# RustAudio/lewton

Hardware: NVIDIA H100
Metric: Msamples/s IMDCT+window+OLA, 2048-pt long blocks (higher is better)
Workload: dtype f32

## Files before the change

lewton_b200/build.py:

```python
import os
import re
import shutil
import subprocess

HERE = os.path.dirname(os.path.abspath(__file__))
CSRC = os.path.join(HERE, "csrc")
SO = os.path.join(HERE, "liblewton_b200.so")
K_LONG_REGS = 249
SOURCES = ["lwb_api.cu", "host_objects.cuh", "path_generic.cuh", "path_long.cuh", "path_chain.cuh", "path_mixed.cuh", "path_mid.cuh",
           "tables_host.cpp", "frontend.cpp", "batcher_submit.cpp", "batcher.h", "lwb_common.h", "pcm_copy_plan.h", "kernels_generic.cuh", "kernel_long.cuh", "kernel_deal.cuh", "kernel_short.cuh", "kernel_mid.cuh", "kernel_chain.cuh", "kernel_prologue.cuh", "kernel_floor0.cuh", "floor1_eval.cuh",
           "floor1_inverse_db.inc", "Makefile"]


def _stale():
    if not os.path.exists(SO):
        return True
    t = os.path.getmtime(SO)
    deps = [os.path.join(CSRC, s) for s in SOURCES] + [os.path.join(HERE, "..", "include", h)
                                                       for h in ("lewton_b200.h", "lewton_frontend.h")]
    return any(os.path.getmtime(d) > t for d in deps)


def check_no_fma(so=SO):
    if shutil.which("cuobjdump") is None:
# ... 41 lines not shown
```

lewton_b200/csrc/host_objects.cuh:

```cuda
#pragma once

struct DevBuf {
    void *p = nullptr;
    size_t cap = 0;
};

struct Staging {
    void *h = nullptr;
    size_t cap = 0;
    cudaEvent_t ev = nullptr;
    bool pending = false;
};

struct ArenaSet {
    DevBuf coeffs, dense, pcm, kinds, ys, vqoff, vqrec;
    cudaEvent_t done = nullptr;
};
constexpr int kHostSets = 2;

struct CachedTables {
    DevTables dt;
    std::vector<float> a, b, c, w;
    std::vector<uint32_t> br;
    std::vector<void *> allocs;
// ... 7 lines not shown
    cudaEvent_t ev_in[64] = {}, ev_done[65] = {};
    DevBuf runs_buf[2];
    cudaEvent_t ev_desc[2] = {}, ev_kdone[2] = {};
    int runs_par = 0;
    uint32_t ticket_next = 0;
    uint64_t epoch = 0;
    uint64_t state_gen = 1;
    std::string err;
    uint64_t launches = 0;
    uint64_t kernel_launches[LWB_KERNEL_COUNT] = {};
    std::vector<PcmSpan> pcm_spans;
    std::vector<PcmCopy> pcm_copies;
    std::deque<CachedTables> tables;
    DevBuf spec, segtab, magic, x, desc, chains, ticket, cdesc, cbytes;
    DevBuf floor0;
    ArenaSet host_sets[kHostSets];
    int host_next = 0;
    ArenaSet ordered;
    Staging stage[3];
    int stage_next = 0;
    std::vector<void *> stage_old;
    uint64_t tickets_issued = 0, tickets_done = 0;
    std::deque<cudaEvent_t> ticket_events;
    std::vector<cudaEvent_t> spare_events;
    size_t x_cap_elems = (size_t)64 << 20;
};

struct lwb_setup {
    lwb_ctx *ctx = nullptr;
    DevSetup host;
    DevSetup *d_setup = nullptr;
    std::vector<void *> allocs;
    uint8_t channels = 0, bs0 = 0, bs1 = 0;
    uint32_t n_modes = 0;
    uint32_t n_mappings = 0;
    std::vector<DevMapping> mappings;
    std::vector<uint8_t> floor_types;
    std::vector<DevFloor0> floor0;
    mutable bool streams_opened = false;
    bool floor0_described(uint32_t fi) const { return fi < floor0.size() && floor0[fi].order != 0; }
    unsigned out_channels() const { return host.n_out ? host.n_out : channels; }
};

struct RowCopy { const float *src; float *dst; uint32_t n4, pad; };
struct ChainShape { unsigned warps; size_t smem; int n1max, wpc, np; };

struct Step {
    int kernel;
    const void *desc;
    size_t n;
    const float *pack;
};

struct StepArgs {
    void *pcm = nullptr;
    int out_format = LWB_OUT_F32_PLANAR;
    const float *w_short = nullptr;
    int ls = 0;
    int mid_kb = 0;
// ... 28 lines not shown
    lwb_batch_io io;
    bool captured = false;
    uint64_t gen = 0;
    FrontStages front;
    DevBuf pro, desc;
    StepArgs args;
    std::vector<Step> steps;
};

struct lwb_stream {
    lwb_ctx *ctx = nullptr;
    const lwb_setup *setup = nullptr;
    float *d_state = nullptr;
    bool has = false;
    uint32_t plen = 0;
    uint64_t busy_epoch = 0;
};

static void capture(lwb_plan *plan, uint64_t gen, const FrontStages &front, const StepArgs &args, std::vector<Step> steps)
{
    plan->captured = true;
    plan->gen = gen;
    plan->front = front;
    for (size_t i = 0; i < plan->n_chains && front.n; i++)
        if (!plan->chains[i].stream->setup->floor0.empty()) plan->front.floor0 = true;
    plan->args = args;
    plan->steps = std::move(steps);
}


static inline void set_stream_state(lwb_stream *s, bool has, uint32_t plen)
{
    if (s->has != has || s->plen != plen) {
        s->has = has;
        s->plen = plen;
        s->ctx->state_gen++;
    }
}

static int fail(lwb_ctx *ctx, int code, const char *what, cudaError_t e = cudaSuccess)
{
    if (ctx) {
        ctx->err = what;
        if (e != cudaSuccess) {
            ctx->err += ": ";
            ctx->err += cudaGetErrorString(e);
        }
    }
    return code;
}
// ... 190 lines not shown
```

lewton_b200/csrc/kernel_long.cuh:

```cuda
#pragma once
#include <stdint.h>

#include "lwb_common.h"

#if defined(__CUDACC__)
#include <cuda_fp16.h>
#include <cuda_runtime.h>

#include <type_traits>
#define LWB_HD __host__ __device__ __forceinline__
#else
#define LWB_HD inline
#endif

namespace lwb {

constexpr int kLongBs = 11;
constexpr int kLongN = 2048;
constexpr int kLongN2 = 1024;

struct alignas(16) LongRun {
    const float *in;
    void *out;
    float *state;
    uint32_t in_stride;
    uint32_t n_packets;
    uint8_t has_prev;
    uint8_t write_state;
    uint8_t dummy;
    uint8_t first_short;
    uint8_t last_short;
    uint8_t pad[3];
    float *state_out;
};
static_assert(sizeof(LongRun) == 48, "LongRun is copied by TMA in 16-byte units");

struct V { float x, y; };

#if defined(__CUDA_ARCH__)
__device__ __forceinline__ V vadd(V a, V b) { return V{__fadd_rn(a.x, b.x), __fadd_rn(a.y, b.y)}; }
__device__ __forceinline__ V vsub(V a, V b) { return V{__fsub_rn(a.x, b.x), __fsub_rn(a.y, b.y)}; }
__device__ __forceinline__ V vmul(V a, V b) { return V{__fmul_rn(a.x, b.x), __fmul_rn(a.y, b.y)}; }
__device__ __forceinline__ V vadd_p(V a, V b) { return V{__fadd_rn(a.x, b.x), __fadd_rn(a.y, b.y)}; }
__device__ __forceinline__ V vsub_p(V a, V b) { return V{__fsub_rn(a.x, b.x), __fsub_rn(a.y, b.y)}; }
__device__ __forceinline__ V vnsub_p(V a, V b) { return V{__fsub_rn(-a.x, b.x), __fsub_rn(-a.y, b.y)}; }
#else
inline V vadd(V a, V b) { return V{a.x + b.x, a.y + b.y}; }
// ... 351 lines not shown
__device__ __forceinline__ void mbar_wait(uint32_t bar, uint32_t parity)
{
    asm volatile(
        "{\n\t.reg .pred p;\n\t"
        "WAIT_%=:\n\t"
        "mbarrier.try_wait.parity.shared::cta.b64 p, [%0], %1, %2;\n\t"
        "@p bra DONE_%=;\n\t"
        "bra WAIT_%=;\n\t"
        "DONE_%=:\n\t}" ::"r"(bar), "r"(parity), "r"(200000u) : "memory");
}
__device__ __forceinline__ void tma_load_1d(uint32_t dst, const void *src, uint32_t bytes, uint32_t bar)
{
    asm volatile("cp.async.bulk.shared::cluster.global.mbarrier::complete_tx::bytes [%0], [%1], %2, [%3];"
                 ::"r"(dst), "l"(src), "r"(bytes), "r"(bar) : "memory");
}
__device__ __forceinline__ void fence_proxy_async()
{
    asm volatile("fence.proxy.async.shared::cta;" ::: "memory");
}
__device__ __forceinline__ void sts_eo(uint32_t addr, float e, float o)
{
    asm volatile("st.shared.f32 [%0], %1;\n\tst.shared.f32 [%0+2048], %2;" ::"r"(addr), "f"(e), "f"(o) : "memory");
}
__device__ __forceinline__ void lds_eo(uint32_t addr, float &e, float &o)
{
    asm volatile("ld.shared.f32 %0, [%2];\n\tld.shared.f32 %1, [%2+2048];" : "=f"(e), "=f"(o) : "r"(addr) : "memory");
}

}
#include "kernel_deal.cuh"
// ... 22 lines not shown
#define LWB_KA(j) (4u * (uint32_t)swz(64 * (j)))
#define LWB_KB(j, h) (4u * (uint32_t)swz(((h) << 6) | ((j) << 3)))
#define LWB_KC(j) (4u * (uint32_t)swz(j))

struct RunCur {
    const float *in;
    void *out;
    float *state;
    uint32_t in_stride;
    uint32_t flags;
};
__device__ __forceinline__ RunCur run_cur(const LongRun &r)
{
    return RunCur{r.in, r.out, r.state, r.in_stride,
                  (uint32_t)(r.has_prev ? 1u : 0u) | (r.write_state ? 2u : 0u) | (r.dummy ? 4u : 0u) |
                      (r.first_short ? 8u : 0u) | (r.last_short ? 16u : 0u)};
}
struct RunCurS : RunCur { float *state_out; };
__device__ __forceinline__ RunCurS run_cur_s(const LongRun &r)
{
    RunCurS c;
    static_cast<RunCur &>(c) = run_cur(r);
    c.flags |= r.first_short == 2 ? 32u : 0u;
    c.state_out = r.state_out ? r.state_out : r.state;
    return c;
}

__device__ __forceinline__ int16_t d_sample_i16(float v)
{
    short r;
    asm("cvt.rzi.s16.f32 %0, %1;" : "=h"(r) : "f"(__fmul_rn(v, 32768.0f)));
// ... 12 lines not shown
__device__ __forceinline__ void st_pcm(int16_t *p, float v) { __stcs(reinterpret_cast<short *>(p), (short)d_sample_i16(v)); }
__device__ __forceinline__ void st_pcm(__half *p, float v) { __stcs(reinterpret_cast<short *>(p), __half_as_short(d_sample_f16(v))); }

template <SampleKind K>
using sample_t = std::conditional_t<K == kSampleF32, float, std::conditional_t<K == kSampleI16, int16_t, __half>>;

template <int FORMAT>
__device__ __forceinline__ void store_sample(void *pcm, uint64_t off, uint64_t stride, unsigned channels, unsigned ch,
                                             uint64_t i, float v)
{
    constexpr OutFormat F = out_format_of(FORMAT);
    using T = sample_t<F.kind>;
    static_cast<T *>(pcm)[off + (F.planar ? (uint64_t)ch * stride + i : i * channels + ch)] = d_sample(v, static_cast<T *>(nullptr));
}

template <int NB, bool FIRST, typename OutT, typename RC = RunCur>
__device__ __forceinline__ void out_stage(const TwMix &tw, int lane, const V O[NB][8], const V E[NB][8], V pe[NB][8],
                                          const RC cur[NB], OutT *out[NB], const float *s_state)
{
#pragma unroll
    for (int j = 0; j < 8; j++) {
        const int r64 = 64 * rev3(j);
        const bool nat = (j & 1);
        const V b0 = tw(P_B0 + j), b1 = tw(P_B1 + j);
        const V wlo = tw(P_WLO + j), whi = tw(P_WHI + j);
#pragma unroll
        for (int b = 0; b < NB; b++) {
            V plo = pe[b][j], phi = pe[b][j];
            bool emit = !(cur[b].flags & 4u);
            if (FIRST) {
                emit = emit && (cur[b].flags & 1u);
                if (cur[b].flags & 1u) {
                    const float *s_lo = s_state + b * kLongN2 + lane, *s_hi = s_state + b * kLongN2 + 63 - lane;
                    const float ax = nat ? s_lo[r64] : s_hi[r64], ay = nat ? s_hi[r64] : s_lo[r64];
                    const float bx = nat ? s_hi[960 - r64] : s_lo[960 - r64];
                    const float by = nat ? s_lo[960 - r64] : s_hi[960 - r64];
                    plo = V{ax, ay};
                    phi = V{bx, by};
                }
            }
            V lo, hi, pev;
            step8_ola(b0, b1, wlo, whi, O[b][j], E[b][j], plo, phi, lo, hi, pev);
            pe[b][j] = pev;
            if (emit) {
                OutT *o_lo = out[b] + lane, *o_hi = out[b] + 63 - lane;
                if (nat) {
                    st_pcm(o_lo + r64, lo.x); st_pcm(o_hi + r64, lo.y);
                    st_pcm(o_hi + 960 - r64, hi.x); st_pcm(o_lo + 960 - r64, hi.y);
                } else {
                    st_pcm(o_hi + r64, lo.x); st_pcm(o_lo + r64, lo.y);
                    st_pcm(o_lo + 960 - r64, hi.x); st_pcm(o_hi + 960 - r64, hi.y);
                }
            }
// ... 113 lines not shown
        const uint32_t bar = bars_s + 8 * stage;
        mbar_expect_tx(bar, kLongStageBytes);
#pragma unroll
        for (int b = 0; b < NB; b++)
            tma_load_1d(tiles_s + stage * kLongStageBytes + b * kLongTileBytes,
                        r[b].in + (size_t)pkt * r[b].in_stride, kLongTileBytes, bar);
    };
    auto issue_stage_cur = [&](uint32_t stage, uint32_t pkt) {
        const uint32_t bar = bars_s + 8 * stage;
        mbar_expect_tx(bar, kLongStageBytes);
#pragma unroll
        for (int b = 0; b < NB; b++)
            tma_load_1d(tiles_s + stage * kLongStageBytes + b * kLongTileBytes,
                        cur[b].in + (size_t)pkt * cur[b].in_stride, kLongTileBytes, bar);
    };
    auto issue_state = [&](const float *const st[NB], const uint32_t has[NB]) {
        uint32_t bytes = 0;
#pragma unroll
        for (int b = 0; b < NB; b++) bytes += has[b] ? kLongTileBytes : 0;
        mbar_expect_tx(bar_state, bytes);
#pragma unroll
        for (int b = 0; b < NB; b++)
            if (has[b]) tma_load_1d(state_s + b * kLongTileBytes, st[b], kLongTileBytes, bar_state);
    };

    {
        uint32_t idx = 0;
        if (lane == 0) idx = atomicAdd(ticket, 1u);
        idx = __shfl_sync(0xffffffffu, idx, 0);
        if (idx >= n_groups) return;
#pragma unroll
        for (int b = 0; b < NB; b++) cur[b] = run_cur(runs[idx * NB + b]);
        npk = runs[idx * NB].n_packets;
        if (lane == 0) {
            fence_proxy_async();
            const float *st[NB];
            uint32_t has[NB];
#pragma unroll
            for (int b = 0; b < NB; b++) { st[b] = cur[b].state; has[b] = cur[b].flags & 1u; }
            issue_state(st, has);
            for (; lc < (uint32_t)kLongRing && lc < npk; lc++) issue_stage_cur(lc, lc);
            nx_idx = atomicAdd(ticket, 1u);
        }
    }

    for (;;) {
        V pe[NB][8];
#pragma unroll
        for (int b = 0; b < NB; b++)
#pragma unroll
            for (int j = 0; j < 8; j++) pe[b][j] = V{0.f, 0.f};
        OutT *out[NB];
#pragma unroll
        for (int b = 0; b < NB; b++) out[b] = static_cast<OutT *>(cur[b].out);

// ... 85 lines not shown
                            issue_stage(tgt, s_next, nx_lc);
                            nx_lc++;
                        }
                    }
                }
            }
            phase_c_fft<NB>(tw, O, E);
            if (p > 0) {
                out_stage<NB, false, OutT>(tw, lane, O, E, pe, cur, out, s_state);
            } else {
                mbar_wait(bar_state, (phase_bits >> 30) & 1u);
                phase_bits ^= 1u << 30;
                if (NB == 1 && (cur[0].flags & 8u))
                    out_first_short<NB, OutT>(tw, lane, O, E, pe, cur, out, s_state, w_short, ls);
                else
                    out_stage<NB, true, OutT>(tw, lane, O, E, pe, cur, out, s_state);
                __syncwarp();
            }
#pragma unroll
            for (int b = 0; b < NB; b++)
                if (p > 0 || (cur[b].flags & 1u)) out[b] += (p == 0 && (cur[b].flags & 8u)) ? kLongN2 - ls : kLongN2;
            if (lane == 0 && nx_stage == 2 && !nx_state_issued) {
                const float *st[NB];
                uint32_t has[NB];
#pragma unroll
                for (int b = 0; b < NB; b++) { st[b] = s_next[b].state; has[b] = s_next[b].has_prev; }
                fence_proxy_async();
                issue_state(st, has);
                nx_state_issued = 1;
            }
            slot_i = (slot_i + 1 == (uint32_t)kLongRing) ? 0 : slot_i + 1;
        }
#pragma unroll
        for (int b = 0; b < NB; b++) {
            if ((cur[b].flags & 16u)) {
                const bool emitted = (npk > 1 || (cur[b].flags & 1u)) && !(cur[b].flags & 4u);
                const bool keep = (cur[b].flags & 6u) == 2u;
#pragma unroll
                for (int j = 0; j < 8; j++) {
                    const int r64 = 64 * rev3(j);
#pragma unroll
                    for (int h = 0; h < 2; h++) {
                        const float v = ((j & 1) != 0) == (h == 0) ? pe[b][j].x : pe[b][j].y;
                        const int m = r64 + (h ? 63 - lane : lane);
                        if (m < ls) {
                            if (emitted) st_pcm(out[b] + m, v);
                        } else if (keep && m < kLongN2 - ls) {
                            cur[b].state[m - ls] = v;
                            cur[b].state[kLongN2 - 1 - ls - m] = v;
                        }
                    }
                }
            } else if ((cur[b].flags & 6u) == 2u) {
                float *s_lo = cur[b].state + lane, *s_hi = cur[b].state + 63 - lane;
#pragma unroll
                for (int j = 0; j < 8; j++) {
                    const int r64 = 64 * rev3(j);
                    const float vx = (j & 1) ? pe[b][j].x : pe[b][j].y, vy = (j & 1) ? pe[b][j].y : pe[b][j].x;
                    s_lo[r64] = vx; s_hi[r64] = vy;
                    s_hi[960 - r64] = vx; s_lo[960 - r64] = vy;
                }
            }
        }
        uint32_t st_ = 0, nlc = 0;
        if (lane == 0) {
            if (nx_stage == 0) {
                if (nx_idx < n_groups) {
                    fence_proxy_async();
                    mbar_expect_tx(bar_desc, NB * (uint32_t)sizeof(LongRun));
                    tma_load_1d(next_s, runs + (size_t)nx_idx * NB, NB * (uint32_t)sizeof(LongRun), bar_desc);
                    nx_stage = 1;
                } else {
                    nx_stage = 3;
                }
            }
            if (nx_stage == 1) {
                mbar_wait(bar_desc, desc_parity);
                desc_parity ^= 1u;
                nx_stage = 2;
                nx_npk = s_next[0].n_packets;
                nx_lc = 0;
            }
            if (nx_stage == 2 && !nx_state_issued) {
                const float *st[NB];
                uint32_t has[NB];
#pragma unroll
                for (int b = 0; b < NB; b++) { st[b] = s_next[b].state; has[b] = s_next[b].has_prev; }
                fence_proxy_async();
                issue_state(st, has);
            }
            st_ = nx_stage;
            nlc = nx_lc;
        }
        st_ = __shfl_sync(0xffffffffu, st_, 0);
        nlc = __shfl_sync(0xffffffffu, nlc, 0);
        if (st_ != 2) break;
        __syncwarp();
#pragma unroll
        for (int b = 0; b < NB; b++) cur[b] = run_cur(s_next[b]);
        npk = s_next[0].n_packets;
        __syncwarp();
        lc = nlc;
        nx_stage = 0; nx_lc = 0; nx_npk = 0; nx_state_issued = 0;
        if (lane == 0) {
// ... 244 lines not shown
```

lewton_b200/csrc/lwb_api.cu:

```cuda
#include <cuda_runtime.h>
#include <sched.h>
#include <sys/syscall.h>
#include <unistd.h>

#include <algorithm>
#include <cctype>
#include <cmath>
#include <cstdio>
#include <cstdlib>
#include <cstring>
#include <deque>
#include <new>
#include <string>
#include <vector>

#include "kernel_long.cuh"
#include "kernel_short.cuh"
#include "kernel_mid.cuh"
#include "kernels_generic.cuh"
#include "kernel_chain.cuh"
#include "kernel_prologue.cuh"
#include "kernel_floor0.cuh"
#include "lwb_common.h"
#include "pcm_copy_plan.h"
// ... 65 lines not shown
{
    cudaError_t e = cudaStreamSynchronize(ctx->stream);
    for (cudaStream_t s : {ctx->copy_in, ctx->copy_out}) {
        const cudaError_t e2 = s ? cudaStreamSynchronize(s) : cudaSuccess;
        if (e == cudaSuccess) e = e2;
    }
    return e;
}

extern "C" void lwb_ctx_destroy(lwb_ctx *ctx)
{
    if (!ctx) return;
    cudaSetDevice(ctx->device);
    sync_all_streams(ctx);
    for (DevBuf *b : {&ctx->spec, &ctx->segtab, &ctx->magic, &ctx->x, &ctx->desc, &ctx->chains, &ctx->ticket, &ctx->runs_buf[0],
                      &ctx->runs_buf[1], &ctx->cdesc, &ctx->cbytes, &ctx->floor0})
        if (b->p) cudaFree(b->p);
    auto free_set = [](ArenaSet &s) {
        for (DevBuf *b : {&s.coeffs, &s.dense, &s.pcm, &s.kinds, &s.ys, &s.vqoff, &s.vqrec})
            if (b->p) cudaFree(b->p);
        if (s.done) cudaEventDestroy(s.done);
    };
    for (ArenaSet &s : ctx->host_sets) free_set(s);
    free_set(ctx->ordered);
    for (cudaEvent_t e : ctx->ticket_events) cudaEventDestroy(e);
    for (cudaEvent_t e : ctx->spare_events) cudaEventDestroy(e);
    for (CachedTables &ct : ctx->tables)
        for (void *p : ct.allocs) cudaFree(p);
    for (void *h : ctx->stage_old) cudaFreeHost(h);
    for (Staging &st : ctx->stage) {
        if (st.h) cudaFreeHost(st.h);
// ... 432 lines not shown
}

extern "C" void lwb_stream_destroy(lwb_stream *s)
{
    if (!s) return;
    cudaSetDevice(s->ctx->device);
    sync_all_streams(s->ctx);
    cudaFree(s->d_state);
    delete s;
}

extern "C" int lwb_stream_reset(lwb_stream *s)
{
    if (!s) return LWB_ERR_INVALID;
    set_stream_state(s, false, 0);
    return LWB_OK;
}
extern "C" int lwb_stream_is_empty(const lwb_stream *s) { return (!s || !s->has) ? 1 : 0; }
extern "C" uint32_t lwb_stream_state_len(const lwb_stream *s) { return (s && s->has) ? s->plen : 0; }

extern "C" int lwb_stream_clone(const lwb_stream *s, lwb_stream **out)
{
    if (!s || !out) return LWB_ERR_INVALID;
    int rc = lwb_stream_open(s->ctx, s->setup, out);
    if (rc) return rc;
    (*out)->has = s->has;
    (*out)->plen = s->plen;
    lwb_ctx *ctx = s->ctx;
    CU(ctx, cudaMemcpyAsync((*out)->d_state, s->d_state,
                            s->setup->channels * state_stride(s->setup) * sizeof(float),
                            cudaMemcpyDeviceToDevice, ctx->stream));
    return LWB_OK;
}

extern "C" int lwb_stream_export_state(lwb_stream *s, float *out)
{
    if (!s || !out) return LWB_ERR_INVALID;
    if (!s->has) return LWB_OK;
    lwb_ctx *ctx = s->ctx;
    CU(ctx, cudaSetDevice(ctx->device));
    CU(ctx, cudaMemcpy2DAsync(out, s->plen * sizeof(float), s->d_state, state_stride(s->setup) * sizeof(float),
                              s->plen * sizeof(float), s->setup->channels, cudaMemcpyDeviceToHost, ctx->stream));
    CU(ctx, cudaStreamSynchronize(ctx->stream));
    return LWB_OK;
}

extern "C" int lwb_stream_import_state(lwb_stream *s, const float *data, uint32_t len)
{
    if (!s || (!data && len)) return LWB_ERR_INVALID;
    if (len > state_stride(s->setup)) return LWB_ERR_BUFFER;
    lwb_ctx *ctx = s->ctx;
    CU(ctx, cudaSetDevice(ctx->device));
    if (len) {
        CU(ctx, cudaMemcpy2DAsync(s->d_state, state_stride(s->setup) * sizeof(float), data, len * sizeof(float),
                                  len * sizeof(float), s->setup->channels, cudaMemcpyHostToDevice, ctx->stream));
        CU(ctx, cudaStreamSynchronize(ctx->stream));
    }
    s->ctx->state_gen++;
    s->has = true;
    s->plen = len;
    return LWB_OK;
}

extern "C" int lwb_decoded_sample_count(const lwb_setup *su, uint8_t mode, int prev_flag, int next_flag,
                                        uint32_t *n_samples)
{
    if (!su || !n_samples) return LWB_ERR_INVALID;
    Geom g;
    int rc = geometry(su, mode, prev_flag, next_flag, &g);
    if (rc) return rc;
    *n_samples = g.rs - g.ls;
    return LWB_OK;
}

#include "path_generic.cuh"
#include "path_long.cuh"
#include "path_chain.cuh"
#include "path_mixed.cuh"
#include "path_mid.cuh"

using BatchPath = int (*)(lwb_ctx *, const lwb_chain *, size_t, const lwb_batch_io *, const BatchWalk &, bool *, lwb_plan *);
static constexpr BatchPath kBatchPaths[] = {try_long, try_mid, try_mixed, try_chain, try_generic};
constexpr size_t kChainPath = 3, kGenericPath = 4;
static_assert(kBatchPaths[kChainPath] == try_chain && kBatchPaths[kGenericPath] == try_generic && std::size(kBatchPaths) == kGenericPath + 1,
              "kChainPath / kGenericPath name the chain-kernel and the four-kernel path, the last one");

static size_t first_batch_path()
{
    const char *fg = getenv("LWB_FORCE_GENERIC");
    if (!fg) return 0;
    return std::strcmp(fg, "1") == 0 ? kGenericPath : kChainPath;
}

static int check_batch_args(lwb_ctx *ctx, const lwb_chain *chains, size_t n_chains, const lwb_batch_io *io)
{
    if (io->entry != LWB_ENTRY_SPECTRUM && io->entry != LWB_ENTRY_RESIDUE && io->entry != LWB_ENTRY_VQ) return fail(ctx, LWB_ERR_INVALID, "bad entry");
    if (io->memory != LWB_MEM_HOST && io->memory != LWB_MEM_DEVICE) return fail(ctx, LWB_ERR_INVALID, "bad memory space");
    if (!out_format_known(io->out_format)) return fail(ctx, LWB_ERR_INVALID, "bad out_format");
    if (n_chains == 0) return LWB_OK;
    if ((!io->coeffs && io->entry != LWB_ENTRY_VQ) || !io->pcm) return fail(ctx, LWB_ERR_INVALID, "null arena");
// ... 56 lines not shown
}

static int queue_batch(lwb_ctx *ctx, lwb_chain *chains, size_t n_chains, const lwb_batch_io *io, lwb_plan *prepared, bool pinned_only)
{
    if (!ctx || (!chains && n_chains) || !io) return LWB_ERR_INVALID;
    BatchWalk bw;
    int rc = walk_batch(ctx, chains, n_chains, io, pinned_only, &bw);
    if (rc || n_chains == 0) return rc;
    CU(ctx, cudaSetDevice(ctx->device));
    if (prepared) prepared->captured = false;
    size_t first = first_batch_path();
    for (size_t i = 0; i < n_chains && first < kChainPath; i++)
        if (chains[i].stream->setup->host.n_out) first = kChainPath;
    for (size_t k = first; k < std::size(kBatchPaths); k++) {
        bool handled = false;
        if ((rc = kBatchPaths[k](ctx, chains, n_chains, io, bw, &handled, prepared))) return rc;
        if (!handled) continue;
        for (size_t i = 0; i < n_chains; i++) set_chain_result(&chains[i], bw.walks[i]);
        commit_stream_states(chains, bw.walks);
        return LWB_OK;
    }
    return fail(ctx, LWB_ERR_INVALID, "internal: no batch path took the batch");
}

static int decode_chains_impl(lwb_ctx *ctx, lwb_chain *chains, size_t n_chains, const lwb_batch_io *io, lwb_plan *prepared,
                              uint64_t *ticket = nullptr)
{
    if (!ctx) return LWB_ERR_INVALID;
    const uint64_t issued = ctx->tickets_issued;
    int rc = queue_batch(ctx, chains, n_chains, io, prepared, ticket != nullptr);
    if (rc) return rc;
    if (!ticket) return ctx->tickets_issued != issued ? retire_tickets(ctx, ctx->tickets_issued, true) : LWB_OK;
    if (ctx->tickets_issued == issued) {
        CU(ctx, cudaSetDevice(ctx->device));
// ... 219 lines not shown
```

lewton_b200/csrc/path_chain.cuh:

```cuda
#pragma once

static size_t chain_smem(unsigned maxc, int n1max, int np, bool vq = false)
{
    return (size_t)maxc * ((size_t)np * n1max + n1max / 2) * 4 + 8 * (LWB_MAX_POSTS + 1) * 2 * 2 + 64 +
           (vq ? (size_t)maxc * (n1max / 2) * 4 : 0);
}
static int chain_np(unsigned maxc, int n1max, int wpc, bool residue)
{
    if (residue || wpc != 1) return 1;
    int np = 4;
    while (np > 1 && chain_smem(maxc, n1max, np) > 64 * 1024) np >>= 1;
    return np;
}
static ChainShape chain_shape(unsigned maxc, int n1max, bool residue, bool vq = false)
{
    int wpc = std::max(1, std::min(8, n1max / 1024));
    while (wpc > 1 && (unsigned)wpc * maxc > 32) wpc >>= 1;
    const int np = chain_np(maxc, n1max, wpc, residue);
    return ChainShape{maxc * wpc, chain_smem(maxc, n1max, np, vq), n1max, wpc, np};
}

__global__ void k_row_copy(const RowCopy *__restrict__ rc)
{
    const RowCopy c = rc[blockIdx.x];
    for (uint32_t i = threadIdx.x; i < c.n4; i += blockDim.x)
        reinterpret_cast<float4 *>(c.dst)[i] = reinterpret_cast<const float4 *>(c.src)[i];
}

static void chain_desc(const lwb_chain *c, uint32_t p0, uint32_t n, bool has, uint32_t plen, uint64_t coeff, uint64_t pos, uint32_t byte_off,
                       ChainDesc *d)
{
    const lwb_stream *s = c->stream;
    const lwb_setup *su = s->setup;
    std::memset(d, 0, sizeof(*d));
    d->setup = su->d_setup;
    d->state = s->d_state;
    d->coeff_off = coeff;
    d->out_off = c->out_offset + pos;
    d->out_stride = c->out_stride;
    d->pkt_index = c->packet_index + p0;
    d->n_packets = n;
// ... 99 lines not shown
```

lewton_b200/csrc/path_long.cuh:

```cuda
#pragma once

struct LongItem {
    const lwb_chain *c;
    uint32_t P;
    bool has_prev;
};

static void long_runs_of(const LongItem &it, size_t cuts, const float *coeffs, char *pcm, size_t esz, LongRun *&w)
{
    for (unsigned ch = 0; ch < it.c->stream->setup->channels; ch++, w += cuts)
        channel_run(it.c, ch, kLongN2, coeffs + it.c->coeff_offset, pcm, esz, it.P, it.has_prev, it.has_prev ? kLongN2 : 0, cuts, w);
}

static bool batch_is_uniform_long(const lwb_chain *chains, size_t n_chains, const lwb_batch_io *io, const BatchWalk &bw)
{
    if (!fused_layout(chains, n_chains, io)) return false;
    const float *pack = nullptr;
    for (size_t i = 0; i < n_chains; i++) {
        const lwb_chain *c = &chains[i];
        const lwb_stream *s = c->stream;
        const lwb_setup *su = s->setup;
        if (su->bs1 != kLongBs || !su->host.tab[1].pack) return false;
        if (pack && pack != su->host.tab[1].pack) return false;
        pack = su->host.tab[1].pack;
        if (s->has && s->plen != (uint32_t)kLongN2) return false;
        if (bw.walks[i].done != c->n_packets || !bw.walks[i].long_only) return false;
    }
    return true;
}

struct LongRuns {
    struct Chunk { size_t r0, nr; };
    std::vector<Chunk> chunks;
    Staging *st = nullptr;
    LongRun *h = nullptr, *d = nullptr;
    size_t n = 0;
    int par = 0;
    bool own = false;
};

static int long_build_runs(lwb_ctx *ctx, const lwb_chain *chains, size_t n_chains, size_t n_chunks, const float *coeffs, char *pcm,
                           size_t esz, DevBuf *own, LongRuns *lr)
{
    std::vector<LongItem> items;
    items.reserve(n_chains);
    size_t chan_chains = 0;
    for (size_t i = 0; i < n_chains; i++) {
        const lwb_chain *c = &chains[i];
        items.push_back(LongItem{c, c->n_packets, c->stream->has});
        if (c->n_packets) chan_chains += c->stream->setup->channels;
    }
    const size_t warp_slots = (size_t)ctx->sm_count * kLongWarps * kLongNB;
    size_t target_runs = warp_slots * 4;
    if (const char *e = getenv("LWB_LONG_TARGET_RUNS")) target_runs = (size_t)atol(e);
    const size_t min_run = 8;
    int rc;
    std::vector<size_t> cuts(items.size(), 1);
    size_t total_runs = 0;
    for (size_t i = 0; i < items.size(); i++) {
        if (!items[i].P) { cuts[i] = 0; continue; }
        const size_t per_launch = std::max<size_t>(1, chan_chains / n_chunks);
        size_t k = 1;
        if (per_launch < target_runs) k = (target_runs + per_launch - 1) / per_launch;
        cuts[i] = std::max<size_t>(1, std::min(k, items[i].P / min_run));
// ... 11 lines not shown
    lr->h = h_runs;
    std::vector<LongRun> tmp;
    std::vector<uint32_t> order;
    for (size_t k = 0; k < n_chunks; k++) {
        const size_t i0 = items.size() * k / n_chunks, i1 = items.size() * (k + 1) / n_chunks;
        LongRun *w0 = w;
        size_t chunk_runs = 0;
        for (size_t i = i0; i < i1; i++)
            if (items[i].P) chunk_runs += cuts[i] * items[i].c->stream->setup->channels;
        LongRun *gen = w;
        if (kLongNB > 1) {
            tmp.resize(chunk_runs);
            gen = tmp.data();
        }
        for (size_t i = i0; i < i1; i++)
            if (items[i].P) long_runs_of(items[i], cuts[i], coeffs, pcm, esz, gen);
        if (kLongNB == 1) {
            w = gen;
        } else {
            bool sorted = true;
            for (size_t i = 1; i < tmp.size() && sorted; i++) sorted = tmp[i].n_packets == tmp[0].n_packets;
            order.resize(tmp.size());
            for (uint32_t i = 0; i < order.size(); i++) order[i] = i;
            if (!sorted)
                std::stable_sort(order.begin(), order.end(),
                                 [&](uint32_t a, uint32_t b) { return tmp[a].n_packets < tmp[b].n_packets; });
            size_t i = 0;
            while (i < order.size()) {
                size_t j = i;
                while (j < order.size() && tmp[order[j]].n_packets == tmp[order[i]].n_packets) j++;
                for (size_t q = i; q < j; q++) *w++ = tmp[order[q]];
// ... 60 lines not shown
    StepArgs args;
    args.pcm = ar.pcm;
    args.out_format = io->out_format;
    std::vector<Step> steps;
    LongRuns lr;
    uint64_t gen = 0;
    size_t pk0 = 0;
    for (size_t k = 0; k < n_chunks; k++) {
        const size_t i0 = n_chains * k / n_chunks, i1 = n_chains * (k + 1) / n_chunks;
        const BatchExtent ke = chunk_extent(io, chains, bw, i0, i1);
        if (ke.empty()) continue;
        size_t npk = 0;
        for (size_t i = i0; i < i1; i++) npk += chains[i].n_packets;
        if ((rc = ar.upload(k, ke)) || (residue && (rc = front_stages_launch(ctx, ar, fs, pk0, npk)))) return rc;
        if (!lr.d) {
            if ((rc = long_build_runs(ctx, chains, n_chains, n_chunks, in, ar.pcm, out_format_of(io->out_format).esz, cap ? &plan->desc : nullptr, &lr)) ||
                (rc = long_upload_runs(ctx, lr, host ? ctx->copy_in : ctx->copy_out)))
                return rc;
            gen = ctx->state_gen;
        }
        steps.assign(1, Step{LWB_KERNEL_LONG, lr.d + lr.chunks[k].r0, lr.chunks[k].nr / kLongNB, pack});
        if ((rc = run_steps(ctx, args, steps)) || (rc = ar.download(k, chains, bw, i0, i1, ke))) return rc;
        pk0 += npk;
    }
    CU(ctx, cudaEventRecord(ctx->ev_kdone[lr.par], ctx->stream));
    if (cap) capture(plan, gen, fs, args, std::move(steps));
    return ar.finish();
}
```

Before: 322,400.

## Store long-block overlap state packed as half row with L2 evict-last hints

```diff
diff --git a/lewton_b200/build.py b/lewton_b200/build.py
--- a/lewton_b200/build.py
+++ b/lewton_b200/build.py
@@ -6,7 +6,7 @@
 HERE = os.path.dirname(os.path.abspath(__file__))
 CSRC = os.path.join(HERE, "csrc")
 SO = os.path.join(HERE, "liblewton_b200.so")
-K_LONG_REGS = 249
+K_LONG_REGS = 251
 SOURCES = ["lwb_api.cu", "host_objects.cuh", "path_generic.cuh", "path_long.cuh", "path_chain.cuh", "path_mixed.cuh", "path_mid.cuh",
            "tables_host.cpp", "frontend.cpp", "batcher_submit.cpp", "batcher.h", "lwb_common.h", "pcm_copy_plan.h", "kernels_generic.cuh", "kernel_long.cuh", "kernel_deal.cuh", "kernel_short.cuh", "kernel_mid.cuh", "kernel_chain.cuh", "kernel_prologue.cuh", "kernel_floor0.cuh", "floor1_eval.cuh",
            "floor1_inverse_db.inc", "Makefile"]
diff --git a/lewton_b200/csrc/host_objects.cuh b/lewton_b200/csrc/host_objects.cuh
--- a/lewton_b200/csrc/host_objects.cuh
+++ b/lewton_b200/csrc/host_objects.cuh
@@ -45,6 +45,7 @@
     std::deque<CachedTables> tables;
     DevBuf spec, segtab, magic, x, desc, chains, ticket, cdesc, cbytes;
     DevBuf floor0;
+    DevBuf expand;
     ArenaSet host_sets[kHostSets];
     int host_next = 0;
     ArenaSet ordered;
@@ -73,7 +74,7 @@
     unsigned out_channels() const { return host.n_out ? host.n_out : channels; }
 };
 
-struct RowCopy { const float *src; float *dst; uint32_t n4, pad; };
+struct RowCopy { const float *src; float *dst; uint32_t n4, mirror; };
 struct ChainShape { unsigned warps; size_t smem; int n1max, wpc, np; };
 
 struct Step {
@@ -132,6 +133,7 @@
     float *d_state = nullptr;
     bool has = false;
     uint32_t plen = 0;
+    bool packed = false;
     uint64_t busy_epoch = 0;
 };
 
@@ -152,6 +154,14 @@
     if (s->has != has || s->plen != plen) {
         s->has = has;
         s->plen = plen;
+        s->ctx->state_gen++;
+    }
+}
+
+static inline void set_stream_packed(lwb_stream *s, bool packed)
+{
+    if (s->packed != packed) {
+        s->packed = packed;
         s->ctx->state_gen++;
     }
 }
diff --git a/lewton_b200/csrc/kernel_long.cuh b/lewton_b200/csrc/kernel_long.cuh
--- a/lewton_b200/csrc/kernel_long.cuh
+++ b/lewton_b200/csrc/kernel_long.cuh
@@ -30,7 +30,9 @@
     uint8_t dummy;
     uint8_t first_short;
     uint8_t last_short;
-    uint8_t pad[3];
+    uint8_t state_in_packed;
+    uint8_t state_out_packed;
+    uint8_t pad;
     float *state_out;
 };
 static_assert(sizeof(LongRun) == 48, "LongRun is copied by TMA in 16-byte units");
@@ -412,6 +414,21 @@
     asm volatile("cp.async.bulk.shared::cluster.global.mbarrier::complete_tx::bytes [%0], [%1], %2, [%3];"
                  ::"r"(dst), "l"(src), "r"(bytes), "r"(bar) : "memory");
 }
+__device__ __forceinline__ uint64_t l2_evict_last()
+{
+    uint64_t p;
+    asm volatile("createpolicy.fractional.L2::evict_last.b64 %0, 1.0;" : "=l"(p));
+    return p;
+}
+__device__ __forceinline__ void tma_load_state(uint32_t dst, const void *src, uint32_t bytes, uint32_t bar)
+{
+    asm volatile("cp.async.bulk.shared::cluster.global.mbarrier::complete_tx::bytes.L2::cache_hint [%0], [%1], %2, [%3], %4;"
+                 ::"r"(dst), "l"(src), "r"(bytes), "r"(bar), "l"(l2_evict_last()) : "memory");
+}
+__device__ __forceinline__ void st_state(float *p, float v, uint64_t policy)
+{
+    asm volatile("st.global.L2::cache_hint.f32 [%0], %1, %2;" ::"l"(p), "f"(v), "l"(policy) : "memory");
+}
 __device__ __forceinline__ void fence_proxy_async()
 {
     asm volatile("fence.proxy.async.shared::cta;" ::: "memory");
@@ -464,7 +481,8 @@
 {
     return RunCur{r.in, r.out, r.state, r.in_stride,
                   (uint32_t)(r.has_prev ? 1u : 0u) | (r.write_state ? 2u : 0u) | (r.dummy ? 4u : 0u) |
-                      (r.first_short ? 8u : 0u) | (r.last_short ? 16u : 0u)};
+                      (r.first_short ? 8u : 0u) | (r.last_short ? 16u : 0u) | (r.state_in_packed ? 64u : 0u) |
+                      (r.state_out_packed ? 128u : 0u)};
 }
 struct RunCurS : RunCur { float *state_out; };
 __device__ __forceinline__ RunCurS run_cur_s(const LongRun &r)
@@ -507,7 +525,7 @@
     static_cast<T *>(pcm)[off + (F.planar ? (uint64_t)ch * stride + i : i * channels + ch)] = d_sample(v, static_cast<T *>(nullptr));
 }
 
-template <int NB, bool FIRST, typename OutT, typename RC = RunCur>
+template <int NB, bool FIRST, typename OutT, typename RC = RunCur, bool PACKED = false>
 __device__ __forceinline__ void out_stage(const TwMix &tw, int lane, const V O[NB][8], const V E[NB][8], V pe[NB][8],
                                           const RC cur[NB], OutT *out[NB], const float *s_state)
 {
@@ -526,10 +544,14 @@
                 if (cur[b].flags & 1u) {
                     const float *s_lo = s_state + b * kLongN2 + lane, *s_hi = s_state + b * kLongN2 + 63 - lane;
                     const float ax = nat ? s_lo[r64] : s_hi[r64], ay = nat ? s_hi[r64] : s_lo[r64];
-                    const float bx = nat ? s_hi[960 - r64] : s_lo[960 - r64];
-                    const float by = nat ? s_lo[960 - r64] : s_hi[960 - r64];
                     plo = V{ax, ay};
-                    phi = V{bx, by};
+                    if (PACKED && (cur[b].flags & 64u)) {
+                        phi = plo;
+                    } else {
+                        const float bx = nat ? s_hi[960 - r64] : s_lo[960 - r64];
+                        const float by = nat ? s_lo[960 - r64] : s_hi[960 - r64];
+                        phi = V{bx, by};
+                    }
                 }
             }
             V lo, hi, pev;
@@ -673,14 +695,15 @@
             tma_load_1d(tiles_s + stage * kLongStageBytes + b * kLongTileBytes,
                         cur[b].in + (size_t)pkt * cur[b].in_stride, kLongTileBytes, bar);
     };
-    auto issue_state = [&](const float *const st[NB], const uint32_t has[NB]) {
-        uint32_t bytes = 0;
-#pragma unroll
-        for (int b = 0; b < NB; b++) bytes += has[b] ? kLongTileBytes : 0;
-        mbar_expect_tx(bar_state, bytes);
+    auto state_bytes = [](uint32_t has, uint32_t packed) { return has ? (packed ? kLongTileBytes / 2 : kLongTileBytes) : 0u; };
+    auto issue_state = [&](const float *const st[NB], const uint32_t bytes[NB]) {
+        uint32_t total = 0;
+#pragma unroll
+        for (int b = 0; b < NB; b++) total += bytes[b];
+        mbar_expect_tx(bar_state, total);
 #pragma unroll
         for (int b = 0; b < NB; b++)
-            if (has[b]) tma_load_1d(state_s + b * kLongTileBytes, st[b], kLongTileBytes, bar_state);
+            if (bytes[b]) tma_load_state(state_s + b * kLongTileBytes, st[b], bytes[b], bar_state);
     };
 
     {
@@ -694,10 +717,10 @@
         if (lane == 0) {
             fence_proxy_async();
             const float *st[NB];
-            uint32_t has[NB];
-#pragma unroll
-            for (int b = 0; b < NB; b++) { st[b] = cur[b].state; has[b] = cur[b].flags & 1u; }
-            issue_state(st, has);
+            uint32_t bytes[NB];
+#pragma unroll
+            for (int b = 0; b < NB; b++) { st[b] = cur[b].state; bytes[b] = state_bytes(cur[b].flags & 1u, cur[b].flags & 64u); }
+            issue_state(st, bytes);
             for (; lc < (uint32_t)kLongRing && lc < npk; lc++) issue_stage_cur(lc, lc);
             nx_idx = atomicAdd(ticket, 1u);
         }
@@ -813,7 +836,7 @@
                 if (NB == 1 && (cur[0].flags & 8u))
                     out_first_short<NB, OutT>(tw, lane, O, E, pe, cur, out, s_state, w_short, ls);
                 else
-                    out_stage<NB, true, OutT>(tw, lane, O, E, pe, cur, out, s_state);
+                    out_stage<NB, true, OutT, RunCur, true>(tw, lane, O, E, pe, cur, out, s_state);
                 __syncwarp();
             }
 #pragma unroll
@@ -821,11 +844,11 @@
                 if (p > 0 || (cur[b].flags & 1u)) out[b] += (p == 0 && (cur[b].flags & 8u)) ? kLongN2 - ls : kLongN2;
             if (lane == 0 && nx_stage == 2 && !nx_state_issued) {
                 const float *st[NB];
-                uint32_t has[NB];
-#pragma unroll
-                for (int b = 0; b < NB; b++) { st[b] = s_next[b].state; has[b] = s_next[b].has_prev; }
+                uint32_t bytes[NB];
+#pragma unroll
+                for (int b = 0; b < NB; b++) { st[b] = s_next[b].state; bytes[b] = state_bytes(s_next[b].has_prev, s_next[b].state_in_packed); }
                 fence_proxy_async();
-                issue_state(st, has);
+                issue_state(st, bytes);
                 nx_state_issued = 1;
             }
             slot_i = (slot_i + 1 == (uint32_t)kLongRing) ? 0 : slot_i + 1;
@@ -852,12 +875,22 @@
                 }
             } else if ((cur[b].flags & 6u) == 2u) {
                 float *s_lo = cur[b].state + lane, *s_hi = cur[b].state + 63 - lane;
-#pragma unroll
-                for (int j = 0; j < 8; j++) {
-                    const int r64 = 64 * rev3(j);
-                    const float vx = (j & 1) ? pe[b][j].x : pe[b][j].y, vy = (j & 1) ? pe[b][j].y : pe[b][j].x;
-                    s_lo[r64] = vx; s_hi[r64] = vy;
-                    s_hi[960 - r64] = vx; s_lo[960 - r64] = vy;
+                if (cur[b].flags & 128u) {
+                    const uint64_t pol = l2_evict_last();
+#pragma unroll
+                    for (int j = 0; j < 8; j++) {
+                        const int r64 = 64 * rev3(j);
+                        const float vx = (j & 1) ? pe[b][j].x : pe[b][j].y, vy = (j & 1) ? pe[b][j].y : pe[b][j].x;
+                        st_state(s_lo + r64, vx, pol); st_state(s_hi + r64, vy, pol);
+                    }
+                } else {
+#pragma unroll
+                    for (int j = 0; j < 8; j++) {
+                        const int r64 = 64 * rev3(j);
+                        const float vx = (j & 1) ? pe[b][j].x : pe[b][j].y, vy = (j & 1) ? pe[b][j].y : pe[b][j].x;
+                        s_lo[r64] = vx; s_hi[r64] = vy;
+                        s_hi[960 - r64] = vx; s_lo[960 - r64] = vy;
+                    }
                 }
             }
         }
@@ -882,11 +915,11 @@
             }
             if (nx_stage == 2 && !nx_state_issued) {
                 const float *st[NB];
-                uint32_t has[NB];
-#pragma unroll
-                for (int b = 0; b < NB; b++) { st[b] = s_next[b].state; has[b] = s_next[b].has_prev; }
+                uint32_t bytes[NB];
+#pragma unroll
+                for (int b = 0; b < NB; b++) { st[b] = s_next[b].state; bytes[b] = state_bytes(s_next[b].has_prev, s_next[b].state_in_packed); }
                 fence_proxy_async();
-                issue_state(st, has);
+                issue_state(st, bytes);
             }
             st_ = nx_stage;
             nlc = nx_lc;
diff --git a/lewton_b200/csrc/lwb_api.cu b/lewton_b200/csrc/lwb_api.cu
--- a/lewton_b200/csrc/lwb_api.cu
+++ b/lewton_b200/csrc/lwb_api.cu
@@ -103,7 +103,7 @@
     cudaSetDevice(ctx->device);
     sync_all_streams(ctx);
     for (DevBuf *b : {&ctx->spec, &ctx->segtab, &ctx->magic, &ctx->x, &ctx->desc, &ctx->chains, &ctx->ticket, &ctx->runs_buf[0],
-                      &ctx->runs_buf[1], &ctx->cdesc, &ctx->cbytes, &ctx->floor0})
+                      &ctx->runs_buf[1], &ctx->cdesc, &ctx->cbytes, &ctx->floor0, &ctx->expand})
         if (b->p) cudaFree(b->p);
     auto free_set = [](ArenaSet &s) {
         for (DevBuf *b : {&s.coeffs, &s.dense, &s.pcm, &s.kinds, &s.ys, &s.vqoff, &s.vqrec})
@@ -566,6 +566,7 @@
 {
     if (!s) return LWB_ERR_INVALID;
     set_stream_state(s, false, 0);
+    set_stream_packed(s, false);
     return LWB_OK;
 }
 extern "C" int lwb_stream_is_empty(const lwb_stream *s) { return (!s || !s->has) ? 1 : 0; }
@@ -582,6 +583,7 @@
     CU(ctx, cudaMemcpyAsync((*out)->d_state, s->d_state,
                             s->setup->channels * state_stride(s->setup) * sizeof(float),
                             cudaMemcpyDeviceToDevice, ctx->stream));
+    (*out)->packed = s->packed;
     return LWB_OK;
 }
 
@@ -591,9 +593,12 @@
     if (!s->has) return LWB_OK;
     lwb_ctx *ctx = s->ctx;
     CU(ctx, cudaSetDevice(ctx->device));
+    const uint32_t n = s->packed ? s->plen / 2 : s->plen;
     CU(ctx, cudaMemcpy2DAsync(out, s->plen * sizeof(float), s->d_state, state_stride(s->setup) * sizeof(float),
-                              s->plen * sizeof(float), s->setup->channels, cudaMemcpyDeviceToHost, ctx->stream));
+                              n * sizeof(float), s->setup->channels, cudaMemcpyDeviceToHost, ctx->stream));
     CU(ctx, cudaStreamSynchronize(ctx->stream));
+    for (unsigned ch = 0; ch < s->setup->channels && s->packed; ch++)
+        for (uint32_t m = 0; m < n; m++) out[(size_t)ch * s->plen + s->plen - 1 - m] = out[(size_t)ch * s->plen + m];
     return LWB_OK;
 }
 
@@ -611,6 +616,7 @@
     s->ctx->state_gen++;
     s->has = true;
     s->plen = len;
+    s->packed = false;
     return LWB_OK;
 }
 
@@ -633,9 +639,39 @@
 
 using BatchPath = int (*)(lwb_ctx *, const lwb_chain *, size_t, const lwb_batch_io *, const BatchWalk &, bool *, lwb_plan *);
 static constexpr BatchPath kBatchPaths[] = {try_long, try_mid, try_mixed, try_chain, try_generic};
-constexpr size_t kChainPath = 3, kGenericPath = 4;
-static_assert(kBatchPaths[kChainPath] == try_chain && kBatchPaths[kGenericPath] == try_generic && std::size(kBatchPaths) == kGenericPath + 1,
-              "kChainPath / kGenericPath name the chain-kernel and the four-kernel path, the last one");
+constexpr size_t kLongPath = 0, kChainPath = 3, kGenericPath = 4;
+static_assert(kBatchPaths[kLongPath] == try_long && kBatchPaths[kChainPath] == try_chain && kBatchPaths[kGenericPath] == try_generic &&
+                  std::size(kBatchPaths) == kGenericPath + 1,
+              "kLongPath / kChainPath / kGenericPath name the fused long-block, the chain-kernel and the four-kernel path, the last one");
+
+static int expand_packed_states(lwb_ctx *ctx, lwb_stream *const *streams, size_t n)
+{
+    std::vector<RowCopy> rows;
+    for (size_t i = 0; i < n; i++)
+        for (unsigned ch = 0; streams[i]->packed && ch < streams[i]->setup->channels; ch++) {
+            float *row = streams[i]->d_state + (size_t)ch * state_stride(streams[i]->setup);
+            rows.push_back(RowCopy{row, row + kLongN2 / 2, kLongN2 / 8, 1});
+        }
+    if (rows.empty()) return LWB_OK;
+    const size_t bytes = rows.size() * sizeof(RowCopy);
+    Staging *st;
+    int rc;
+    if ((rc = ensure(ctx, ctx->expand, bytes)) || (rc = acquire_staging(ctx, bytes, &st))) return rc;
+    std::memcpy(st->h, rows.data(), bytes);
+    if ((rc = upload_staging(ctx, st, st->h, ctx->expand.p, bytes, ctx->stream)) ||
+        (rc = launch(ctx, LWB_KERNEL_ROW_COPY, k_row_copy, dim3((unsigned)rows.size()), dim3(64), 0, (const RowCopy *)ctx->expand.p)))
+        return rc;
+    for (size_t i = 0; i < n; i++) set_stream_packed(streams[i], false);
+    return LWB_OK;
+}
+
+static int expand_batch_states(lwb_ctx *ctx, const lwb_chain *chains, size_t n_chains)
+{
+    std::vector<lwb_stream *> packed;
+    for (size_t i = 0; i < n_chains; i++)
+        if (chains[i].stream->packed) packed.push_back(chains[i].stream);
+    return expand_packed_states(ctx, packed.data(), packed.size());
+}
 
 static size_t first_batch_path()
 {
@@ -722,10 +758,15 @@
         if (chains[i].stream->setup->host.n_out) first = kChainPath;
     for (size_t k = first; k < std::size(kBatchPaths); k++) {
         bool handled = false;
-        if ((rc = kBatchPaths[k](ctx, chains, n_chains, io, bw, &handled, prepared))) return rc;
+        if ((k != kLongPath && (rc = expand_batch_states(ctx, chains, n_chains))) ||
+            (rc = kBatchPaths[k](ctx, chains, n_chains, io, bw, &handled, prepared)))
+            return rc;
         if (!handled) continue;
         for (size_t i = 0; i < n_chains; i++) set_chain_result(&chains[i], bw.walks[i]);
         commit_stream_states(chains, bw.walks);
+        if (k == kLongPath)
+            for (size_t i = 0; i < n_chains; i++)
+                if (bw.walks[i].done) set_stream_packed(chains[i].stream, long_packs_state(prepared, io));
         return LWB_OK;
     }
     return fail(ctx, LWB_ERR_INVALID, "internal: no batch path took the batch");
diff --git a/lewton_b200/csrc/path_chain.cuh b/lewton_b200/csrc/path_chain.cuh
--- a/lewton_b200/csrc/path_chain.cuh
+++ b/lewton_b200/csrc/path_chain.cuh
@@ -23,8 +23,16 @@
 __global__ void k_row_copy(const RowCopy *__restrict__ rc)
 {
     const RowCopy c = rc[blockIdx.x];
-    for (uint32_t i = threadIdx.x; i < c.n4; i += blockDim.x)
-        reinterpret_cast<float4 *>(c.dst)[i] = reinterpret_cast<const float4 *>(c.src)[i];
+    const float4 *src = reinterpret_cast<const float4 *>(c.src);
+    float4 *dst = reinterpret_cast<float4 *>(c.dst);
+    for (uint32_t i = threadIdx.x; i < c.n4; i += blockDim.x) {
+        if (c.mirror) {
+            const float4 v = src[c.n4 - 1 - i];
+            dst[i] = make_float4(v.w, v.z, v.y, v.x);
+        } else {
+            dst[i] = src[i];
+        }
+    }
 }
 
 static void chain_desc(const lwb_chain *c, uint32_t p0, uint32_t n, bool has, uint32_t plen, uint64_t coeff, uint64_t pos, uint32_t byte_off,
diff --git a/lewton_b200/csrc/path_long.cuh b/lewton_b200/csrc/path_long.cuh
--- a/lewton_b200/csrc/path_long.cuh
+++ b/lewton_b200/csrc/path_long.cuh
@@ -4,12 +4,20 @@
     const lwb_chain *c;
     uint32_t P;
     bool has_prev;
+    bool packed;
 };
 
-static void long_runs_of(const LongItem &it, size_t cuts, const float *coeffs, char *pcm, size_t esz, LongRun *&w)
-{
-    for (unsigned ch = 0; ch < it.c->stream->setup->channels; ch++, w += cuts)
+static bool long_packs_state(const lwb_plan *plan, const lwb_batch_io *io) { return plan && io->memory == LWB_MEM_DEVICE; }
+
+static void long_runs_of(const LongItem &it, size_t cuts, const float *coeffs, char *pcm, size_t esz, bool pack, LongRun *&w)
+{
+    for (unsigned ch = 0; ch < it.c->stream->setup->channels; ch++, w += cuts) {
         channel_run(it.c, ch, kLongN2, coeffs + it.c->coeff_offset, pcm, esz, it.P, it.has_prev, it.has_prev ? kLongN2 : 0, cuts, w);
+        for (size_t k = 0; k < cuts; k++) {
+            w[k].state_in_packed = w[k].has_prev && it.packed;
+            w[k].state_out_packed = pack;
+        }
+    }
 }
 
 static bool batch_is_uniform_long(const lwb_chain *chains, size_t n_chains, const lwb_batch_io *io, const BatchWalk &bw)
@@ -40,14 +48,14 @@
 };
 
 static int long_build_runs(lwb_ctx *ctx, const lwb_chain *chains, size_t n_chains, size_t n_chunks, const float *coeffs, char *pcm,
-                           size_t esz, DevBuf *own, LongRuns *lr)
+                           size_t esz, bool pack, DevBuf *own, LongRuns *lr)
 {
     std::vector<LongItem> items;
     items.reserve(n_chains);
     size_t chan_chains = 0;
     for (size_t i = 0; i < n_chains; i++) {
         const lwb_chain *c = &chains[i];
-        items.push_back(LongItem{c, c->n_packets, c->stream->has});
+        items.push_back(LongItem{c, c->n_packets, c->stream->has, c->stream->packed});
         if (c->n_packets) chan_chains += c->stream->setup->channels;
     }
     const size_t warp_slots = (size_t)ctx->sm_count * kLongWarps * kLongNB;
@@ -89,7 +97,7 @@
             gen = tmp.data();
         }
         for (size_t i = i0; i < i1; i++)
-            if (items[i].P) long_runs_of(items[i], cuts[i], coeffs, pcm, esz, gen);
+            if (items[i].P) long_runs_of(items[i], cuts[i], coeffs, pcm, esz, pack, gen);
         if (kLongNB == 1) {
             w = gen;
         } else {
@@ -180,7 +188,8 @@
         for (size_t i = i0; i < i1; i++) npk += chains[i].n_packets;
         if ((rc = ar.upload(k, ke)) || (residue && (rc = front_stages_launch(ctx, ar, fs, pk0, npk)))) return rc;
         if (!lr.d) {
-            if ((rc = long_build_runs(ctx, chains, n_chains, n_chunks, in, ar.pcm, out_format_of(io->out_format).esz, cap ? &plan->desc : nullptr, &lr)) ||
+            if ((rc = long_build_runs(ctx, chains, n_chains, n_chunks, in, ar.pcm, out_format_of(io->out_format).esz, long_packs_state(plan, io),
+                                     cap ? &plan->desc : nullptr, &lr)) ||
                 (rc = long_upload_runs(ctx, lr, host ? ctx->copy_in : ctx->copy_out)))
                 return rc;
             gen = ctx->state_gen;
diff --git a/profiles/state_traffic_bench.py b/profiles/state_traffic_bench.py
--- /dev/null
+++ b/profiles/state_traffic_bench.py
@@ -0,0 +1,109 @@
+#!/usr/bin/env python3
+import argparse
+import json
+import os
+import subprocess
+import sys
+
+ROOT = os.path.dirname(os.path.dirname(os.path.abspath(__file__)))
+N2, C = 1024, 2
+
+
+def card():
+    q = "name,power.limit,clocks.sm,clocks.max.sm"
+    try:
+        out = subprocess.run(["nvidia-smi", "--id=0", f"--query-gpu={q}", "--format=csv,noheader"], capture_output=True,
+                             text=True, check=True).stdout.strip()
+    except (OSError, subprocess.CalledProcessError) as e:
+        raise SystemExit(f"nvidia-smi failed: {e}: this measurement needs the GPU")
+    return dict(zip(q.split(","), (v.strip() for v in out.split(","))))
+
+
+def child(args):
+    sys.path.insert(0, ROOT)
+    import numpy as np
+    import torch
+
+    import lewton_b200 as L
+    from lewton_b200 import _cabi as cabi
+    torch.cuda.set_device(0)
+    ctx = L.Context(0)
+    su = L.Setup(ctx, C, 8, 11, [L.FloorTypeOne(1, [0, 128])], [L.Mapping(C)], [L.ModeInfo(False), L.ModeInfo(True)])
+    stream = torch.cuda.ExternalStream(ctx.cuda_stream, device=torch.device("cuda", 0))
+    gen = torch.Generator(device="cuda").manual_seed(1234)
+    res = {}
+    for P in args.packets:
+        S = args.streams
+        spec = torch.randn((S, P, C, N2), generator=gen, device="cuda", dtype=torch.float32) * 1e-2
+        pcm = torch.empty((S, C, P * N2), device="cuda", dtype=torch.float32)
+        pwrs = [L.PreviousWindowRight(su) for _ in range(S)]
+        chains = [L.ChainSpec(pwrs[s], np.ones(P, np.uint8), coeff_offset=s * P * C * N2, out_offset=s * C * P * N2,
+                              out_stride=P * N2) for s in range(S)]
+        batch = L.Batch(ctx, chains, cabi.ENTRY_SPECTRUM, cabi.MEM_DEVICE, spec.data_ptr(), pcm.data_ptr(), cabi.OUT_F32_PLANAR)
+        for _ in range(5):
+            batch.run()
+        ctx.synchronize()
+        steps = max(20, int(args.seconds * 1e3 / (0.03 * P)))
+        e0, e1 = torch.cuda.Event(enable_timing=True), torch.cuda.Event(enable_timing=True)
+        e0.record(stream)
+        for _ in range(steps):
+            batch.run()
+        e1.record(stream)
+        ctx.synchronize()
+        ms = e0.elapsed_time(e1) / steps
+        alg = S * P * C * N2 * 8
+        state = S * C * 2 * args.row_bytes
+        res[P] = {"ms_per_step": ms, "alg_bytes": alg, "state_bytes": state, "total_gbs": (alg + state) / (ms * 1e-3) / 1e9,
+                  "alg_gbs": alg / (ms * 1e-3) / 1e9, "msamples_s": S * P * C * N2 / (ms * 1e-3) / 1e6, "steps": steps}
+        batch.close()
+        for p in pwrs:
+            p.close()
+        del spec, pcm
+    ctx.close()
+    print(json.dumps(res))
+
+
+def main():
+    ap = argparse.ArgumentParser()
+    ap.add_argument("--lib", action="append", default=[], metavar="LABEL=PATH:ROWBYTES",
+                    help="a library and the bytes of one state row it reads and writes per run (4096 full, 2048 packed)")
+    ap.add_argument("--rounds", type=int, default=5)
+    ap.add_argument("--streams", type=int, default=4096)
+    ap.add_argument("--packets", type=int, nargs="+", default=[16, 64])
+    ap.add_argument("--seconds", type=float, default=0.5, help="timed window per shape and run")
+    ap.add_argument("--child", action="store_true", help=argparse.SUPPRESS)
+    ap.add_argument("--row-bytes", type=int, default=2048, help=argparse.SUPPRESS)
+    args = ap.parse_args()
+    if args.child:
+        return child(args)
+    libs = []
+    for spec in args.lib or [f"tree={os.path.join(ROOT, 'lewton_b200', 'liblewton_b200.so')}:2048"]:
+        label, rest = spec.split("=", 1)
+        path, row = rest.rsplit(":", 1)
+        libs.append((label, os.path.abspath(path), int(row)))
+    before = card()
+    runs = {label: [] for label, _, _ in libs}
+    for r in range(args.rounds):
+        for label, path, row in (libs if r % 2 == 0 else libs[::-1]):
+            cmd = [sys.executable, os.path.abspath(__file__), "--child", "--row-bytes", str(row), "--streams", str(args.streams),
+                   "--seconds", str(args.seconds), "--packets", *map(str, args.packets)]
+            out = subprocess.run(cmd, env={**os.environ, "LWB_LIB": path}, capture_output=True, text=True)
+            if out.returncode:
+                sys.stderr.write(out.stderr)
+                raise SystemExit(f"{label}: child failed")
+            runs[label].append(json.loads(out.stdout.strip().splitlines()[-1]))
+    summary = {}
+    for label, _, row in libs:
+        summary[label] = {"row_bytes": row}
+        for P in args.packets:
+            ms = sorted(x[str(P)]["ms_per_step"] for x in runs[label])
+            gbs = sorted(x[str(P)]["total_gbs"] for x in runs[label])
+            summary[label][f"P{P}"] = {"ms_median": ms[len(ms) // 2], "ms_range": [ms[0], ms[-1]],
+                                       "total_gbs_median": gbs[len(gbs) // 2], "total_gbs_range": [gbs[0], gbs[-1]],
+                                       "msamples_s_median": sorted(x[str(P)]["msamples_s"] for x in runs[label])[len(ms) // 2]}
+    print(json.dumps({"card_before": before, "card_after": card(), "rounds": args.rounds, "streams": args.streams,
+                      "results": summary, "runs": runs}))
+
+
+if __name__ == "__main__":
+    sys.exit(main())
```

Result: faster. 331,600, median of 6 (+2.9%).
